# WU-CVGL/SIU3R

Measured on AMD Instinct MI355X. Metric: image-pairs/sec @2x512^2 (SIU3R network forward incl. panoptic post-process), higher is better.
Workload: dtype bf16x3 (fp32 activations, bf16 MFMA with hi/lo operand split; meets the 1e-3 parity bar)

## Files before the change

### siu3r_amd/csrc/gemm.hip

```cpp
#include <stdlib.h>

#include "common.h"
#include "gemm_epilogue.h"

int siu3r_gemm_dma_launch(const siu3r_gemm_params& p, int ni, void* stream);
int siu3r_gemm_dma_x3_launch(const siu3r_gemm_params& p, void* stream);
int siu3r_gemm_dma_mode(const siu3r_gemm_params& p);
int siu3r_gemm_dma_x3_mode(const siu3r_gemm_params& p);
int siu3r_gemm_pp_mode(const siu3r_gemm_params& p);
void siu3r_gemm_pp_name(const siu3r_gemm_params& p, int cfg, char* buf, int n);
int siu3r_gemm_pp_launch(const siu3r_gemm_params& p, int cfg, void* stream);
int siu3r_gemm_skinny_launch(const siu3r_gemm_params& p, void* stream);
bool siu3r_gemm_pp_folds_skinny(const siu3r_gemm_params& p);
bool siu3r_gemm_pp_a_x3_ok(const siu3r_gemm_params& p);
bool siu3r_gemm_pp_c_x3_ok(const siu3r_gemm_params& p, int cfg);
static const bool g_disable_dma = getenv("SIU3R_GEMM_NO_DMA") != nullptr;
static const int g_narrow_max = getenv("SIU3R_GEMM_NARROW_MAX") ? atoi(getenv("SIU3R_GEMM_NARROW_MAX")) : 0x7fffffff;

namespace {

constexpr int BM = 128, BK = 64;
constexpr int A_TILE_BYTES = BM * BK * 2;

__device__ __forceinline__ int lds_off(int row, int chunk) {
  return row * 128 + ((chunk ^ ((row >> 1) & 7)) << 4);
}

template <int A_F32, int SPLIT, int NI>
struct Regs {
  float4 ra0[A_F32 ? 4 : 1], ra1[A_F32 ? 4 : 1];
  uint4 rab[A_F32 ? 1 : 4];
  uint4 rwh[2 * NI], rwl[SPLIT ? 2 * NI : 1];
};

template <int A_F32, int SPLIT, int NI, bool LNF = false>
__global__ __launch_bounds__(256) void gemm_kernel(const siu3r_gemm_params p) {
  constexpr int BN = 64 * NI;
  constexpr int B_TILE_BYTES = BN * BK * 2;
  constexpr int PLANES = SPLIT ? 2 : 1;
  constexpr int STAGE_BYTES = PLANES * (A_TILE_BYTES + B_TILE_BYTES);
  constexpr int WROWS = 2 * NI;
  constexpr int SMEM_BYTES = 2 * STAGE_BYTES > siu3r_epi::staging_bytes<NI>() ? 2 * STAGE_BYTES : siu3r_epi::staging_bytes<NI>();
  __shared__ __attribute__((aligned(16))) unsigned char smem[SMEM_BYTES];

  const int t = threadIdx.x;
  const int lane = t & 63, wave = t >> 6;
// ... 236 lines not shown
  if (p.splitk <= 1 || NI != 1) p.splitk = 0;
  if (!p.w_lo && p.a_dtype == SIU3R_BF16 && p.a_mode != 2 && !g_disable_dma) {
    const int rc = siu3r_gemm_dma_launch(p, NI, s);
    if (rc <= 0) return rc;
  }
  if (p.w_x3 && NI == 1 && !g_disable_dma) {
    const int rc = siu3r_gemm_dma_x3_launch(p, s);
    if (rc <= 0) return rc;
  }
  p.splitk = 0;
  if (p.ln_stats) {
    if (p.w_lo) hipLaunchKernelGGL((gemm_kernel<1, 1, NI, true>), grid, block, 0, s, p);
    else if (p.a_dtype == SIU3R_F32) hipLaunchKernelGGL((gemm_kernel<1, 0, NI, true>), grid, block, 0, s, p);
    else hipLaunchKernelGGL((gemm_kernel<0, 0, NI, true>), grid, block, 0, s, p);
  } else if (p.w_lo) {
    hipLaunchKernelGGL((gemm_kernel<1, 1, NI>), grid, block, 0, s, p);
  } else if (p.a_dtype == SIU3R_F32) {
    hipLaunchKernelGGL((gemm_kernel<1, 0, NI>), grid, block, 0, s, p);
  } else {
    hipLaunchKernelGGL((gemm_kernel<0, 0, NI>), grid, block, 0, s, p);
  }
  SIU3R_LAUNCH_CHECK("siu3r_gemm");
  return 0;
}

}


static int g_tile_default = getenv("SIU3R_GEMM_PP") ? atoi(getenv("SIU3R_GEMM_PP")) : 0;
static int g_no_skinny = getenv("SIU3R_GEMM_NO_SKINNY") ? 1 : 0;
static int g_no_splitk = getenv("SIU3R_NO_SPLITK") ? atoi(getenv("SIU3R_NO_SPLITK")) : 0;
static int g_no_tuned = getenv("SIU3R_GEMM_NO_TUNED") ? 1 : 0;
static int g_force_skinny = getenv("SIU3R_GEMM_FORCE_SKINNY") ? 1 : 0;
static float g_bf16_pp_hurdle = getenv("SIU3R_GEMM_BF16_PP_HURDLE") ? (float)atof(getenv("SIU3R_GEMM_BF16_PP_HURDLE")) : 1.3f;
extern "C" int siu3r_gemm_tune(int key, int value) {
  if (key == 0) g_tile_default = value;
  else if (key == 1) g_no_skinny = value;
  else if (key == 2) g_no_splitk = value;
  else if (key == 3) g_no_tuned = value;
  else if (key == 4) g_force_skinny = value;
  else return 1;
  return 0;
}

#include "gemm_tuned.h"

namespace {
const siu3r_tuned_entry* tuned_entry(const siu3r_gemm_params& p, bool x3) {
  const int Z = p.batch > 0 ? p.batch : 1, ln = p.ln_stats ? 1 : 0;
  for (const siu3r_tuned_entry* e = kTuned; e->m; ++e)
    if (e->m == p.m && e->n == p.n && e->k == p.k && e->batch == Z && e->a_mode == p.a_mode && e->out_mode == p.out_mode && e->kh == p.kh &&
        e->stride == p.stride && e->x3 == (x3 ? 1 : 0) && e->ln == ln)
      return e;
  return nullptr;
}

struct Cand { int cfg, bm, bn, slots; float t0_x3, t_step_x3, t0_bf, t_step_bf; };
const Cand kCands[] = {{SIU3R_TILE_PP_256x256, 256, 256, 256, 16.3f, 1.18f, 12.1f, 0.80f},
                       {SIU3R_TILE_PP_256x128, 256, 128, 256, 11.7f, 0.65f, 8.5f, 0.47f},
                       {SIU3R_TILE_PP_128x128, 128, 128, 256, 7.8f, 0.40f, 6.5f, 0.30f},
                       {SIU3R_TILE_128x64, 128, 64, 512, 6.2f, 0.46f, 6.8f, 0.31f}};

void plan(const siu3r_gemm_params& p, siu3r_gemm_plan_t& pl) {
  memset(&pl, 0, sizeof(pl));
  const bool x3 = p.w_x3 != nullptr && p.a_dtype == SIU3R_F32;
  const int pp_mode = (g_disable_dma || p.a_mode == 2) ? -1 : siu3r_gemm_pp_mode(p);
  const int dma_mode = g_disable_dma ? -1 : (x3 ? siu3r_gemm_dma_x3_mode(p) : siu3r_gemm_dma_mode(p));
  int force = p.tile_cfg ? p.tile_cfg : g_tile_default;
  const bool may_split = !g_no_splitk && p.splitk != 1 && p.sk_ws && p.sk_cnt;
  int want_s = p.splitk;
  if (force == 0 && !g_no_tuned) {
    if (const siu3r_tuned_entry* e = tuned_entry(p, x3)) {
      force = e->tile_cfg;
      if (e->splitk > 0 && p.splitk == 0) want_s = (e->splitk > 1 && !may_split) ? 1 : e->splitk;
    }
  }
  const int64_t Z = p.batch > 0 ? p.batch : 1;
  const int ksteps = p.kpad / (x3 ? 16 : 32);
  float best_t = 0.f;
  int best = -1, best_s = 1, best_skinny = 0;
  for (int ci = 0; ci < 4; ++ci) {
    const Cand& c = kCands[ci];
    const bool is_pp = c.cfg > 0;
    if (is_pp && pp_mode < 0) continue;
    if (force != 0 && force != c.cfg && !(force > 0 && !is_pp && pp_mode < 0)) continue;
    const int rem = p.m % c.bm;
    const bool skinny_ok = is_pp && !g_no_skinny && p.a_mode == 0 && rem != 0 && rem <= 32 && p.n >= 64;
    for (int sk = (skinny_ok && g_force_skinny) ? 1 : 0; sk <= (skinny_ok ? 1 : 0); ++sk) {
      const int skinny = sk ? rem : 0;
      const int mrows = p.m - skinny;
      const int64_t tiles = (int64_t)((mrows + c.bm - 1) / c.bm) * ((p.n + c.bn - 1) / c.bn) * Z;
      const bool can_split = may_split && (is_pp || (dma_mode >= 0 && c.bn == 64));
      const bool fixed_s = want_s >= 1 && (want_s == 1 || can_split);
      const int smax = fixed_s ? want_s : (can_split ? 8 : 1);
      for (int S = (fixed_s ? want_s : 1); S <= smax; S *= 2) {
        if (S > 1) {
          if (ksteps / S < (is_pp ? 8 : 16) && !fixed_s) break;
          if (tiles * S * c.bm * c.bn > p.sk_ws_floats || tiles > p.sk_cnt_n) break;
          if (tiles >= 2 * c.slots && !fixed_s) break;
        }
        const int64_t wgs = tiles * S;
        const int64_t rounds = (wgs + c.slots - 1) / c.slots;
        float t = rounds * ((x3 ? c.t0_x3 : c.t0_bf) + (float)((ksteps + S - 1) / S) * (x3 ? c.t_step_x3 : c.t_step_bf));
        if (mrows == 0) t = 0.f;
        if (skinny && mrows > 0 && p.kpad <= 2048 && !getenv("SIU3R_GEMM_NO_FOLD")) t += 1.0f + (x3 ? 5.0f : 3.0f) * (float)p.kpad / 1024.f;
        else if (skinny) t += (skinny <= 4 && p.kpad >= 2048 && p.kpad <= 4096) ? 5.0f + (x3 ? 5.0f : 3.0f) * (float)p.kpad / 1024.f : 3.5f + (x3 ? 9.3f : 5.0f) * (float)p.kpad / 1024.f;
        if (S > 1) t += 2.5f + (float)(2.0 * S * tiles * c.bm * c.bn * 4.0 / 5.0e6);
        if (!x3 && is_pp && force == 0) t *= g_bf16_pp_hurdle;
        if (best < 0 || t < best_t) {
          best = ci;
          best_t = t;
          best_s = S;
          best_skinny = skinny;
        }
      }
    }
  }
  if (best < 0) best = 3;
  const Cand& c = kCands[best];
  pl.tile_cfg = c.cfg;
  pl.bm = c.bm;
  pl.bn = c.bn;
  pl.splitk = best_s;
  pl.skinny_rows = best_skinny;
  if (c.cfg < 0) {
    const int64_t tiles128 = (int64_t)((p.m + BM - 1) / BM) * ((p.n + 127) / 128) * Z;
    const bool narrow = (p.n <= 64) || (tiles128 < g_narrow_max && p.n > 64) || p.w_x3 != nullptr;
    pl.bn = narrow ? 64 : 128;
    if (!narrow || dma_mode < 0) pl.splitk = 1;
  }
  if (pl.splitk > 1) {
    const int64_t tiles = (int64_t)((p.m - pl.skinny_rows + pl.bm - 1) / pl.bm) * ((p.n + pl.bn - 1) / pl.bn) * Z;
    pl.ws_floats = tiles * pl.splitk * pl.bm * pl.bn;
    pl.counters = (int32_t)tiles;
  }
  auto tf = [](bool b) { return b ? "true" : "false"; };
  if (c.cfg > 0) {
    siu3r_gemm_pp_name(p, c.cfg, pl.kernel, sizeof(pl.kernel));
// ... 42 lines not shown
  SIU3R_CHECK(p.tile_cfg >= -1 && p.tile_cfg <= 3, "siu3r_gemm: bad tile_cfg %d", p.tile_cfg);
  if (p.bmod > 0) SIU3R_CHECK(p.batch > 0 && p.batch % p.bmod == 0, "siu3r_gemm: batch %d is not a multiple of bmod %d", p.batch, p.bmod);
  return 0;
}

extern "C" int siu3r_gemm_plan(const siu3r_gemm_params* pp, siu3r_gemm_plan_t* out) {
  SIU3R_CHECK(pp && out, "siu3r_gemm_plan: null argument");
  if (int rc = validate_gemm(*pp)) return rc;
  plan(*pp, *out);
  out->a_x3_ok = out->tile_cfg > 0 && siu3r_gemm_pp_a_x3_ok(*pp);
  out->c_x3_ok = out->tile_cfg > 0 && siu3r_gemm_pp_c_x3_ok(*pp, out->tile_cfg);
  return 0;
}

extern "C" int siu3r_gemm(const siu3r_gemm_params* pp, void* stream) {
  const siu3r_gemm_params& p = *pp;
  if (int rc = validate_gemm(p)) return rc;
  siu3r_gemm_plan_t pl;
  plan(p, pl);
  hipStream_t s = (hipStream_t)stream;
  SIU3R_CHECK(!p.a_x3 || (pl.tile_cfg > 0 && siu3r_gemm_pp_a_x3_ok(p)), "siu3r_gemm: a_x3 (pre-split A planes) needs a ping-pong plan, bf16x3 weights, dense A, "
              "k == kpad and lda / batch strides %% 32 == 0 (this block runs %s): query siu3r_gemm_plan_t.a_x3_ok first", pl.kernel);
  SIU3R_CHECK(!p.c_x3 || (pl.tile_cfg > 0 && siu3r_gemm_pp_c_x3_ok(p, pl.tile_cfg)), "siu3r_gemm: c_x3 (output planes) needs a ping-pong plan and the plain fp32 "
              "row-major output form with n %% 64 == 0, ldc / batch strides %% 32 == 0 (this block runs %s): query siu3r_gemm_plan_t.c_x3_ok first", pl.kernel);
  SIU3R_CHECK(p.c || p.c_x3, "siu3r_gemm: null output");
  siu3r_gemm_params q = p;
  q.splitk = pl.splitk;
  if (pl.splitk > 1) SIU3R_CHECK(p.sk_ws && p.sk_cnt && p.sk_ws_floats >= pl.ws_floats && p.sk_cnt_n >= pl.counters,
                                 "siu3r_gemm: split-K workspace too small (%ld floats / %d counters needed)", (long)pl.ws_floats, pl.counters);
  SIU3R_CHECK(!(p.splitk > 1 && pl.splitk != p.splitk), "siu3r_gemm: splitk=%d was requested but %s cannot split K for this problem (it would run %d slice(s)); "
              "request 0 / 1 or another tile_cfg", p.splitk, pl.kernel, pl.splitk);
  if (pl.tile_cfg > 0) {
    q.m_main = pl.skinny_rows > 0 ? p.m - pl.skinny_rows : 0;
    if (!(pl.skinny_rows > 0 && q.m_main == 0)) {
      const int rc = siu3r_gemm_pp_launch(q, pl.tile_cfg, stream);
      if (rc) return rc;
    }
    if (pl.skinny_rows > 0 && !(q.m_main > 0 && siu3r_gemm_pp_folds_skinny(q))) {
      q.splitk = 0;
      return siu3r_gemm_skinny_launch(q, stream);
    }
    return 0;
  }
  return pl.bn == 64 ? launch<1>(q, s) : launch<2>(q, s);
}
```

### siu3r_amd/csrc/gemm_pp.hip

```cpp
#include "gemm_pp_kernel.h"

namespace siu3r_gemm_pp {
template <bool X3, bool LNF>
__global__ __launch_bounds__(512, 2) void gemm_skinny_kernel(const siu3r_gemm_params p) {
#if __HIP_DEVICE_COMPILE__
  __shared__ __attribute__((aligned(16))) unsigned char smem[SKINNY_SMEM_BYTES];
  skinny_rows_body<X3, LNF>(p, smem, blockIdx.x, blockIdx.z);
#endif
}

constexpr int GV_ROWS = 4, GV_KMAX = 4096;
template <bool X3, bool LNF>
__global__ __launch_bounds__(512) void gemm_skinny_gemv_kernel(const siu3r_gemm_params p) {
#if __HIP_DEVICE_COMPILE__
  constexpr int ESZ = X3 ? 4 : 2;
  __shared__ __attribute__((aligned(16))) float s_a[GV_ROWS * GV_KMAX];
  __shared__ __attribute__((aligned(16))) float s_res[GV_ROWS][64];
  __shared__ __attribute__((aligned(16))) unsigned char s_stage[siu3r_epi_pp::WAVE_STAGE_BYTES];
  const int t = threadIdx.x, lane = t & 63;
  const int wave = __builtin_amdgcn_readfirstlane(t >> 6);
  const int M = p.m, N = p.n, K = p.k, kpad = p.kpad;
  const int row0 = p.m_main, R = M - row0, col0 = blockIdx.x * 64, z = blockIdx.z;
  const siu3r_zoff zof = siu3r_batch_offsets(p, z);
  const unsigned char* Ab = (const unsigned char*)p.a + zof.a * ESZ;
// ... 132 lines not shown
  return p.relu_in ? -1 : 2;
}

void siu3r_gemm_pp_name(const siu3r_gemm_params& p, int cfg, char* buf, int n) {
  const bool x3 = p.w_x3 != nullptr && p.a_dtype == SIU3R_F32;
  const int mode = siu3r_gemm_pp_mode(p);
  snprintf(buf, n, "siu3r_gemm_pp::gemm_pp_kernel<%s, %d, %d, %d, %s, %s%s>", x3 ? "true" : "false", cfg == 3 ? 1 : 2, cfg == 1 ? 4 : 2, mode,
           (mode == 1 && p.relu_in) ? "true" : "false", (mode == 0 && p.ln_stats) ? "true" : "false", (x3 && mode <= 1 && p.a_x3) ? ", true" : "");
}

bool siu3r_gemm_pp_a_x3_ok(const siu3r_gemm_params& p) {
  const bool x3 = p.w_x3 != nullptr && p.a_dtype == SIU3R_F32;
  if (!x3 || ((uintptr_t)p.a % 16) != 0 || p.sa % 32 != 0 || p.sa_i % 32 != 0) return false;
  const int mode = siu3r_gemm_pp_mode(p);
  if (mode == 0) return p.k == p.kpad && p.lda % 32 == 0;
  return mode == 1 && p.cin % 32 == 0 && !p.relu_in;
}
bool siu3r_gemm_pp_c_x3_ok(const siu3r_gemm_params& p, int cfg) {
  if (siu3r_epi_pp::g_force_general || siu3r_gemm_pp_mode(p) < 0) return false;
  const int MI_ = cfg == 3 ? 1 : 2;
  const int64_t res_b = p.r_dtype == SIU3R_F32 ? 4 : 2;
  const bool res_ok = !p.residual || (p.r_dtype == SIU3R_F32 && (p.ldr * res_b) % 16 == 0 && ((uintptr_t)p.residual % 16) == 0 && (p.sr * res_b) % 16 == 0 &&
                                       (p.sr_i * res_b) % 16 == 0 && (int64_t)(32 * MI_) * p.ldr < (1 << 28));
  const bool up_ok = !p.up_src || (p.up_dtype == SIU3R_F32 && ((uintptr_t)p.up_src % 16) == 0 && (int64_t)p.m * p.n < (1 << 29));
  return p.out_mode == 0 && up_ok && !p.c_aux && p.c_dtype == SIU3R_F32 && p.n % 64 == 0 && (int64_t)(32 * MI_) * p.ldc < (1 << 28) && res_ok &&
         p.ldc % 32 == 0 && p.sc % 32 == 0 && p.sc_i % 32 == 0 && ((uintptr_t)p.c % 16) == 0 && ((uintptr_t)p.c_x3 % 16) == 0 &&
         p.c_x3_col0 >= 0 && p.c_x3_col0 % 64 == 0;
}

static const bool g_no_fold = getenv("SIU3R_GEMM_NO_FOLD") != nullptr;
bool siu3r_gemm_pp_folds_skinny(const siu3r_gemm_params& p) {
  return !g_no_fold && p.m_main > 0 && p.m_main < p.m && p.a_mode == 0 && p.kpad <= 2048 && siu3r_gemm_pp_mode(p) == 0;
}

int siu3r_gemm_pp_launch(const siu3r_gemm_params& pin, int cfg, void* stream) {
  using namespace siu3r_gemm_pp;
  siu3r_gemm_params p = pin;
  const bool x3 = p.w_x3 != nullptr && p.a_dtype == SIU3R_F32;
  const int mode = siu3r_gemm_pp_mode(p);
  if (mode < 0) return 1;
  const int MI_ = cfg == 3 ? 1 : 2, NJ_ = cfg == 1 ? 4 : 2;
  const int bm = 128 * MI_, bn = 64 * NJ_;
  const int mrows = p.m_main > 0 ? p.m_main : p.m;
  const int tm = (mrows + bm - 1) / bm, tn = (p.n + bn - 1) / bn;
  int best = -1;
  long best_cost = 0;
  for (int gx = 1; gx <= 8; gx *= 2) {
    const int gy = 8 / gx;
    const int rm = (tm + gy - 1) / gy, rn = (tn + gx - 1) / gx;
    const long cost = (long)rm * rn * 1000000 + (long)rm * bm + (long)rn * bn;
    if (best < 0 || cost < best_cost) {
      best = gx;
      best_cost = cost;
    }
  }
  p.map_gx = best;
  p.map_rm = (tm + (8 / best) - 1) / (8 / best);
  p.map_rn = (tn + best - 1) / best;
  dim3 grid(8 * p.map_rm * p.map_rn, p.splitk > 1 ? p.splitk : 1, p.batch > 0 ? p.batch : 1), block(512);
  p.sk_gx = 0;
  if (siu3r_gemm_pp_folds_skinny(p)) {
    p.sk_gx = (int)grid.x;
    grid.x += (unsigned)((p.n + 63) / 64);
  }
  hipStream_t s = (hipStream_t)stream;
  const bool lnf = p.ln_stats != nullptr;
#ifdef SIU3R_PP_MINI
  hipLaunchKernelGGL((gemm_pp_kernel<SIU3R_PP_MINI, false, false>), grid, block, 0, s, p);
#else
  if (cfg == 1) (x3 ? siu3r_gemm_pp_go_t1x : siu3r_gemm_pp_go_t1b)(p, mode, lnf, grid, s);
  else if (cfg == 2) (x3 ? siu3r_gemm_pp_go_t2x : siu3r_gemm_pp_go_t2b)(p, mode, lnf, grid, s);
  else (x3 ? siu3r_gemm_pp_go_t3x : siu3r_gemm_pp_go_t3b)(p, mode, lnf, grid, s);
#endif
  SIU3R_LAUNCH_CHECK("siu3r_gemm(pp)");
  return 0;
}

int siu3r_gemm_skinny_launch(const siu3r_gemm_params& p, void* stream) {
  using namespace siu3r_gemm_pp;
  const bool x3 = p.w_x3 != nullptr && p.a_dtype == SIU3R_F32;
  dim3 grid((p.n + 63) / 64, 1, p.batch > 0 ? p.batch : 1), block(512);
  hipStream_t s = (hipStream_t)stream;
  const bool lnf = p.ln_stats != nullptr;
#ifndef SIU3R_PP_MINI
  const int rows = p.m - p.m_main, esz = x3 ? 4 : 2;
  static const bool no_gemv = getenv("SIU3R_GEMM_NO_GEMV") != nullptr;
  if (!no_gemv && rows >= 1 && rows <= GV_ROWS && p.kpad >= 2048 && p.kpad <= GV_KMAX && p.k % 4 == 0 && ((int64_t)p.lda * esz) % 16 == 0 &&
      ((uintptr_t)p.a % 16) == 0 && (p.sa * esz) % 16 == 0 && (p.sa_i * esz) % 16 == 0) {
    if (x3 && lnf) hipLaunchKernelGGL((gemm_skinny_gemv_kernel<true, true>), grid, block, 0, s, p);
    else if (x3) hipLaunchKernelGGL((gemm_skinny_gemv_kernel<true, false>), grid, block, 0, s, p);
    else if (lnf) hipLaunchKernelGGL((gemm_skinny_gemv_kernel<false, true>), grid, block, 0, s, p);
    else hipLaunchKernelGGL((gemm_skinny_gemv_kernel<false, false>), grid, block, 0, s, p);
    SIU3R_LAUNCH_CHECK("siu3r_gemm(skinny gemv)");
    return 0;
// ... 10 lines not shown
```

### siu3r_amd/csrc/gemm_pp_kernel.h

```cpp
#pragma once
#include <stdlib.h>

#include "common.h"
#include "gemm_epilogue_pp.h"

#ifndef SIU3R_PP_SCHED
#define SIU3R_PP_SCHED 0
#endif

namespace siu3r_gemm_pp {

constexpr unsigned OOB = 0xffffff00u;
constexpr int RSRC_FLAGS = 0x00020000;
constexpr int nstage(int MI, int NJ) { return (MI == 2 && NJ == 4) ? 4 : (MI == 2 ? 6 : 8); }
constexpr int spp(int MI, int NJ) { return (MI == 2 && NJ == 4) ? 1 : 2; }

typedef __attribute__((address_space(3))) void* lds_ptr;
typedef __attribute__((ext_vector_type(4))) unsigned int u32x4;
typedef __attribute__((ext_vector_type(2))) short i16x2;

template <int MI, int NJ>
constexpr int smem_bytes() {
  constexpr int ring = nstage(MI, NJ) * (128 * MI + 64 * NJ) * 64, st = siu3r_epi_pp::staging_bytes();
  return ring > st ? ring : st;
}

#define SIU3R_DS_READ(dst, addr, OFF) asm volatile("ds_read_b128 %0, %1 offset:%2" : "=v"(dst) : "v"(addr), "i"(OFF) : "memory")

constexpr int SKINNY_SMEM_BYTES = 8 * 8192 + siu3r_epi_pp::WAVE_STAGE_BYTES;
template <bool X3, bool LNF>
__device__ __forceinline__ void skinny_rows_body(const siu3r_gemm_params& p, unsigned char* smem, int colgroup, int z) {
#if __HIP_DEVICE_COMPILE__
  constexpr int ESZ = X3 ? 4 : 2;
  const int t = threadIdx.x, lane = t & 63;
  const int wave = __builtin_amdgcn_readfirstlane(t >> 6);
  const int l31 = lane & 31, lh = lane >> 5;
  const int M = p.m, N = p.n, K = p.k, kpad = p.kpad;
  const int row0 = p.m_main, col0 = colgroup * 64;
  const siu3r_zoff zof = siu3r_batch_offsets(p, z);
  const unsigned char* Ab = (const unsigned char*)p.a + zof.a * ESZ;
  const unsigned char* Wb = X3 ? (const unsigned char*)p.w_x3 + zof.w * 4 : (const unsigned char*)p.w_hi + zof.w * 2;
  const int WROW = X3 ? kpad * 4 : kpad * 2;
  __amdgpu_buffer_rsrc_t rA = __builtin_amdgcn_make_buffer_rsrc((void*)Ab, (short)0, (int)(((int64_t)(M - 1) * p.lda + K) * ESZ), RSRC_FLAGS);
  __amdgpu_buffer_rsrc_t rW = __builtin_amdgcn_make_buffer_rsrc((void*)Wb, (short)0, (int)((int64_t)N * WROW), RSRC_FLAGS);
  int m = row0 + l31;
  if (m > M - 1) m = M - 1;
  const unsigned a_voff = (unsigned)((int64_t)m * p.lda * ESZ + lh * (8 * ESZ));
  const bool aps = X3 && p.a_x3 != 0;
  const unsigned a_voff_ps = (unsigned)((int64_t)m * p.lda * ESZ + lh * 16);
  unsigned w_voff[2];
#pragma unroll
  for (int j = 0; j < 2; ++j) {
    int n = col0 + j * 32 + l31;
    if (n > N - 1) n = N - 1;
    w_voff[j] = (unsigned)((int64_t)n * WROW + lh * 16);
  }
// ... 79 lines not shown
  }
  __syncthreads();
  if (wave != 0) return;
#pragma unroll 1
  for (int w = 1; w < 8; ++w) {
#pragma unroll
    for (int j = 0; j < 2; ++j)
#pragma unroll
      for (int qv = 0; qv < 4; ++qv) {
        const float4 v = *(const float4*)(part + ((w * 8 + j * 4 + qv) * 64 + lane) * 4);
        acc[0][j][4 * qv] += v.x;
        acc[0][j][4 * qv + 1] += v.y;
        acc[0][j][4 * qv + 2] += v.z;
        acc[0][j][4 * qv + 3] += v.w;
      }
  }
  siu3r_epi_pp::wave_rows<1, 2, LNF>(p, acc, (float*)(smem + 8 * 8192), row0, col0, M, z, lane);
#endif
}

template <bool X3, int MI, int NJ, int MODE, bool RELU, bool LNF, bool APS = false>
__global__ __launch_bounds__(512, 2) void gemm_pp_kernel(const siu3r_gemm_params p) {
#if __HIP_DEVICE_COMPILE__
  constexpr int BM = 128 * MI, BN = 64 * NJ;
  constexpr int NSTAGE = nstage(MI, NJ), SPP = spp(MI, NJ), PD = NSTAGE - SPP;
  static_assert(NSTAGE % SPP == 0, "a phase uses whole stages");
  constexpr int STAGE_BYTES = (BM + BN) * 64;
  constexpr int A_PCS = MI, W_PCS = NJ / 2, PPW = A_PCS + W_PCS;
  constexpr int ESZ = X3 ? 4 : 2;
  constexpr int KSTEP = X3 ? 16 : 32;
  constexpr int CK = 16 / ESZ;
  static_assert(NJ % 2 == 0, "W pieces are dealt to whole waves");
  static_assert(!APS || (X3 && MODE <= 1 && !RELU), "pre-split A: bf16x3, dense rows or the tap-cursor gather (cin % 32 == 0)");
  __shared__ __attribute__((aligned(1024))) unsigned char smem[smem_bytes<MI, NJ>()];
  static_assert(smem_bytes<MI, NJ>() >= SKINNY_SMEM_BYTES, "the folded remainder-row workgroups use the ring's LDS");

  if constexpr (MODE == 0) {
    if (p.sk_gx > 0 && (int)blockIdx.x >= p.sk_gx) {
      const int cg = (int)blockIdx.x - p.sk_gx;
      if (blockIdx.y == 0 && cg * 64 < p.n) skinny_rows_body<X3, LNF>(p, smem, cg, blockIdx.z);
      return;
    }
  }

  const int t = threadIdx.x;
  const int lane = t & 63;
  const int wave = __builtin_amdgcn_readfirstlane(t >> 6);
  const int grp = wave >> 2;
  const int wm = wave & 3, wn = grp;
  const int l31 = lane & 31, lh = lane >> 5;

  const int M = p.m_main > 0 ? p.m_main : p.m;
  const int N = p.n, K = p.k, kpad = p.kpad;
  const int tiles_m = (M + BM - 1) / BM, tiles_n = (N + BN - 1) / BN;
  const int xcd = (blockIdx.x + blockIdx.z) & 7, li = blockIdx.x >> 3;
  const int map_gx = p.map_gx;
  const int ry = xcd / map_gx, rx = xcd - ry * map_gx;
  const int lm = li / p.map_rn, ln = li - lm * p.map_rn;
  const int tile_m = ry * p.map_rm + lm, tile_n = rx * p.map_rn + ln;
  if (lm >= p.map_rm || tile_m >= tiles_m || tile_n >= tiles_n) return;
  const int z = blockIdx.z;
  const int np_all = kpad / (KSTEP * SPP);
  const int pbase = p.splitk > 1 ? (int)((int64_t)blockIdx.y * np_all / p.splitk) : 0;
  const int np = p.splitk > 1 ? (int)((int64_t)(blockIdx.y + 1) * np_all / p.splitk) - pbase : np_all;
  const int sbase = pbase * SPP, ns = np * SPP;

  const siu3r_zoff zof = siu3r_batch_offsets(p, z);
  const unsigned char* Ab = (const unsigned char*)p.a + zof.a * ESZ;
  const unsigned char* Wb = X3 ? (const unsigned char*)p.w_x3 + zof.w * 4 : (const unsigned char*)p.w_hi + zof.w * 2;
  const int WROW = X3 ? kpad * 4 : kpad * 2;

  const int prow = lane >> 2;
  const int q = (lane & 3) ^ ((lane >> 4) & 3);
  const int cin = p.cin, iw = p.iw, ih = p.ih, kw = p.kw, kh = p.kh;
  const int pad_bias = (MODE != 0) ? (p.pad * iw + p.pad) * cin * ESZ : 0;
  __amdgpu_buffer_rsrc_t rA, rW;
  if (MODE == 0)
    rA = __builtin_amdgcn_make_buffer_rsrc((void*)Ab, (short)0, (int)(((int64_t)(p.m - 1) * p.lda + K) * ESZ), RSRC_FLAGS);
  else
    rA = __builtin_amdgcn_make_buffer_rsrc((void*)(Ab - pad_bias), (short)0, (int)OOB, RSRC_FLAGS);
  rW = __builtin_amdgcn_make_buffer_rsrc((void*)Wb, (short)0, (int)((int64_t)N * WROW), RSRC_FLAGS);

  unsigned a_voff[A_PCS], a_mask[A_PCS];
  int a_iy0[A_PCS], a_ix0[A_PCS];
#pragma unroll
  for (int i = 0; i < A_PCS; ++i) {
    const int r = (wave * A_PCS + i) * 16 + prow;
    int m = tile_m * BM + r;
    const bool row_ok = m < M;
    if (!row_ok) m = M - 1;
    a_voff[i] = a_mask[i] = 0;
    a_iy0[i] = a_ix0[i] = 0;
    if (MODE == 0) {
      a_voff[i] = (unsigned)((int64_t)m * p.lda * ESZ + q * 16 + ((APS && q >= 2) ? 32 : 0));
    } else {
      const int ohw = p.oh * p.ow;
      const int b = m / ohw, rr = m - b * ohw;
      const int oy = rr / p.ow, ox = rr - oy * p.ow;
      const int iy0 = oy * p.stride - p.pad, ix0 = ox * p.stride - p.pad;
      if (MODE == 1) {
        a_voff[i] = (unsigned)((((b * ih + iy0) * iw + ix0) * cin) * ESZ + q * 16 + ((APS && q >= 2) ? 32 : 0) + pad_bias);
        unsigned mk = 0;
        for (int ky = 0; ky < kh; ++ky)
          for (int kx = 0; kx < kw; ++kx)
            if (iy0 + ky >= 0 && iy0 + ky < ih && ix0 + kx >= 0 && ix0 + kx < iw) mk |= 1u << (ky * kw + kx);
        a_mask[i] = row_ok ? mk : 0u;
      } else {
        a_voff[i] = (unsigned)((((b * ih + iy0) * iw + ix0) * cin) * ESZ + pad_bias);
        a_iy0[i] = row_ok ? iy0 : -(1 << 20);
        a_ix0[i] = ix0;
      }
    }
  }
  unsigned w_voff[W_PCS];
#pragma unroll
  for (int i = 0; i < W_PCS; ++i) {
    const int r = (wave * W_PCS + i) * 16 + prow;
    int n = tile_n * BN + r;
    if (n > N - 1) n = N - 1;
    w_voff[i] = (unsigned)((int64_t)n * WROW + q * 16 + ((X3 && q >= 2) ? 32 : 0));
  }
  const bool ktail = kpad > K;
  const int ks_tail0 = K / KSTEP;

  int cur_c0 = 0, cur_kx = 0, cur_toff = 0, cur_row = 0;
  unsigned cur_bit = 1u;
  auto cursor_advance = [&]() {
    cur_c0 += KSTEP;
    cur_toff += APS ? ((cur_c0 & 16) ? 32 : 96) : KSTEP * ESZ;
    if (cur_c0 == cin) {
      cur_c0 = 0;
      cur_bit <<= 1;
      if (++cur_kx == kw) {
        cur_kx = 0;
        cur_row += iw * cin * ESZ;
      }
      cur_toff = cur_row + cur_kx * cin * ESZ;
    }
  };
  int s_c0 = 0, s_kx = 0, s_ky = 0;
  int qs_r = 0, qs_qx = 0, qs_qy = 0;
  if (MODE == 2) {
    const int qq = KSTEP / cin;
    qs_r = KSTEP - qq * cin;
    qs_qy = qq / kw;
    qs_qx = qq - qs_qy * kw;
    const int k0 = q * CK;
    const int tap = k0 / cin;
    s_c0 = k0 - tap * cin;
    s_ky = tap / kw;
    s_kx = tap - s_ky * kw;
  }
  auto state_advance = [&]() {
    s_c0 += qs_r;
    const int carry = s_c0 >= cin ? 1 : 0;
    s_c0 -= carry * cin;
// ... 4 lines not shown
  };

  auto issue_piece = [&](int s, int stage, int k) {
    const int sg = sbase + (s < ns ? s : ns - 1);
    unsigned char* dstA = smem + stage * STAGE_BYTES + wave * (A_PCS * 1024);
    unsigned char* dstW = smem + stage * STAGE_BYTES + BM * 64 + wave * (W_PCS * 1024);
    if (k < A_PCS) {
      const int i = k;
      if (MODE == 0 && APS) {
        __builtin_amdgcn_raw_ptr_buffer_load_lds(rA, (lds_ptr)(dstA + i * 1024), 16, a_voff[i], (sg >> 1) * 128 + (sg & 1) * 32, 0, 0);
      } else if (MODE == 0) {
        unsigned voff = a_voff[i];
        if (ktail && sg >= ks_tail0) voff = (sg * KSTEP + q * CK < K) ? voff : OOB;
        __builtin_amdgcn_raw_ptr_buffer_load_lds(rA, (lds_ptr)(dstA + i * 1024), 16, voff, sg * 64, 0, 0);
      } else if (MODE == 1) {
        const unsigned voff = (a_mask[i] & cur_bit) ? a_voff[i] : OOB;
        __builtin_amdgcn_raw_ptr_buffer_load_lds(rA, (lds_ptr)(dstA + i * 1024), 16, voff, cur_toff, 0, 0);
      } else {
        const int iy = a_iy0[i] + s_ky, ix = a_ix0[i] + s_kx;
        const bool ok = s_ky < kh && (unsigned)iy < (unsigned)ih && (unsigned)ix < (unsigned)iw;
        const unsigned voff = ok ? a_voff[i] + (unsigned)(((s_ky * iw + s_kx) * cin + s_c0) * ESZ) : OOB;
        __builtin_amdgcn_raw_ptr_buffer_load_lds(rA, (lds_ptr)(dstA + i * 1024), 16, voff, 0, 0, 0);
      }
    } else {
      const int i = k - A_PCS;
      const int soffW = X3 ? (sg >> 1) * 128 + (sg & 1) * 32 : sg * 64;
      __builtin_amdgcn_raw_ptr_buffer_load_lds(rW, (lds_ptr)(dstW + i * 1024), 16, w_voff[i], soffW, 0, 0);
    }
    if (k == PPW - 1) {
      if (MODE == 1 && s + 1 < ns) cursor_advance();
      if (MODE == 2 && s + 1 < ns) state_advance();
    }
  };
  auto issue = [&](int s, int stage) {
#pragma unroll
    for (int k = 0; k < PPW; ++k) issue_piece(s, stage, k);
  };

  f32x16 acc[MI][NJ];
#pragma unroll
  for (int i = 0; i < MI; ++i)
#pragma unroll
    for (int j = 0; j < NJ; ++j)
#pragma unroll
      for (int r = 0; r < 16; ++r) acc[i][j][r] = 0.f;

  const unsigned int lds_base = (unsigned int)(size_t)(__attribute__((address_space(3))) unsigned char*)smem;
  const int fsw = (l31 >> 2) & 3;
  const unsigned int rowA = (wm * (32 * MI) + l31) * 64, rowB = BM * 64 + (wn * (32 * NJ) + l31) * 64;
  const unsigned int offA0 = rowA + ((((X3 && !APS) ? 2 * lh : lh) ^ fsw) << 4), offA1 = rowA + ((((X3 && !APS) ? 2 * lh + 1 : 2 + lh) ^ fsw) << 4);
  const unsigned int offB0 = rowB + ((lh ^ fsw) << 4), offB1 = rowB + (((2 + lh) ^ fsw) << 4);

  u32x4 fa[SPP][MI][2], fb[SPP][NJ][2];
  auto read_frags = [&](int u, int stage) {
    const unsigned int sb = lds_base + stage * STAGE_BYTES;
    const unsigned int a0 = sb + offA0, a1 = sb + offA1, b0 = sb + offB0, b1 = sb + offB1;
#define SIU3R_RD_A(I) if constexpr (I < MI) { SIU3R_DS_READ(fa[u][I][0], a0, I * 2048); SIU3R_DS_READ(fa[u][I][1], a1, I * 2048); }
#define SIU3R_RD_B(J) if constexpr (J < NJ) { SIU3R_DS_READ(fb[u][J][0], b0, J * 2048); SIU3R_DS_READ(fb[u][J][1], b1, J * 2048); }
    SIU3R_RD_A(0) SIU3R_RD_A(1)
    SIU3R_RD_B(0) SIU3R_RD_B(1) SIU3R_RD_B(2) SIU3R_RD_B(3)
#undef SIU3R_RD_A
#undef SIU3R_RD_B
  };
  auto wait_frags = [&]() {
    asm volatile("s_waitcnt lgkmcnt(0)" ::: "memory");
#pragma unroll
    for (int u = 0; u < SPP; ++u) {
#pragma unroll
      for (int i = 0; i < MI; ++i) asm volatile("" : "+v"(fa[u][i][0]), "+v"(fa[u][i][1]));
#pragma unroll
      for (int j = 0; j < NJ; ++j) asm volatile("" : "+v"(fb[u][j][0]), "+v"(fb[u][j][1]));
    }
  };
  auto as_frag = [&](u32x4 v) {
    if (!X3 && RELU) {
#pragma unroll
      for (int e = 0; e < 4; ++e) {
        union { unsigned int u; i16x2 h; } x;
        x.u = v[e];
        x.h = __builtin_elementwise_max(x.h, (i16x2){0, 0});
        v[e] = x.u;
      }
    }
    union { u32x4 u; bf16x8 h; } cv;
    cv.u = v;
    return cv.h;
  };

#ifndef SIU3R_PP_DBG
#define SIU3R_PP_DBG 0
#endif
  constexpr int dbg = SIU3R_PP_DBG;
  constexpr bool dma = !(dbg & 1);
  unsigned tsum[8] = {0, 0, 0, 0, 0, 0, 0, 0}, tlast = 0;
  auto tick = [&](int seg) {
    if constexpr ((dbg & 64) != 0) {
      const unsigned now = (unsigned)__builtin_readcyclecounter();
      tsum[seg] += now - tlast;
      tlast = now;
    }
  };

  for (int s_ = 0; s_ < sbase; ++s_) {
    if (MODE == 1) cursor_advance();
    if (MODE == 2) state_advance();
  }
  constexpr int YOUNG = (PD - SPP) * PPW;
  auto wait_young = [&]() {
    static_assert(YOUNG == 8 || YOUNG == 6, "vmcnt immediate");
    if constexpr (YOUNG == 8) asm volatile("s_waitcnt vmcnt(8)" ::: "memory");
    else asm volatile("s_waitcnt vmcnt(6)" ::: "memory");
  };
  constexpr bool IMF = SIU3R_PP_SCHED == 1;
  const int pd_grp = (IMF && grp == 1) ? PD + SPP : PD;
#pragma unroll
  for (int s_ = 0; s_ < PD; ++s_) issue(s_, s_);
  if (IMF && grp == 1) {
#pragma unroll
    for (int s_ = PD; s_ < PD + SPP; ++s_) issue(s_, s_);
    static_assert(PD * PPW == 12, "vmcnt immediate");
    asm volatile("s_waitcnt vmcnt(12)" ::: "memory");
  } else {
    wait_young();
  }
  __builtin_amdgcn_s_barrier();
  asm volatile("" ::: "memory");
  if (grp == 1) __builtin_amdgcn_s_barrier();
  if constexpr ((dbg & 64) != 0) tlast = (unsigned)__builtin_readcyclecounter();

  int st_rd = 0, st_is = pd_grp % NSTAGE;
  auto mf_hook = [&](int s, int u, int c) {
    if constexpr (IMF) {
      constexpr int TOT = (X3 ? 3 : 2) * MI * NJ;
#pragma unroll
      for (int k = 0; k < PPW; ++k)
        if (dma && c == ((2 * k + 1) * TOT) / (2 * PPW) + 1) {
          issue_piece(s + pd_grp + u, st_is + u, k);
          __builtin_amdgcn_sched_barrier(0);
        }
    }
  };
  for (int s = 0; s < ns; s += SPP) {
    tick(7);
#pragma unroll
    for (int u = 0; u < SPP; ++u)
      if (!(dbg & 4)) read_frags(u, st_rd + u);
    if (dma && !IMF) {
#pragma unroll
      for (int u = 0; u < SPP; ++u) issue(s + PD + u, st_is + u);
    }
    __builtin_amdgcn_sched_barrier(0);
    tick(1);
    wait_frags();
    tick(2);
    if (grp == 1 && dma) wait_young();
    __builtin_amdgcn_sched_barrier(0);
    if (!(dbg & 16)) __builtin_amdgcn_s_barrier();
    __builtin_amdgcn_sched_barrier(0);
    tick(4);
    __builtin_amdgcn_s_setprio(1);
#pragma unroll
    for (int u = 0; u < SPP; ++u) {
      bf16x8 bh[NJ][2];
#pragma unroll
      for (int j = 0; j < NJ; ++j) {
        union { u32x4 u; bf16x8 h; } c0, c1;
        c0.u = fb[u][j][0];
        c1.u = fb[u][j][1];
        bh[j][0] = c0.h;
        bh[j][1] = c1.h;
      }
      if constexpr ((dbg & 2) != 0) {
#pragma unroll
        for (int i = 0; i < MI; ++i) asm volatile("" :: "v"(fa[u][i][0]), "v"(fa[u][i][1]));
#pragma unroll
        for (int j = 0; j < NJ; ++j) asm volatile("" :: "v"(bh[j][0]), "v"(bh[j][1]));
      } else if constexpr (X3) {
        union U8 { u32x4 u; bf16x8 h; };
        U8 ah[MI], al[MI];
        auto raw = [&](int i, int e) { return e < 4 ? fa[u][i][0][e] : fa[u][i][1][e - 4]; };
        auto relu = [&](unsigned int x) { return (RELU && (x & 0x80000000u)) ? 0u : x; };
        auto hi_pair = [&](int i, int e) { ah[i].u[e] = __builtin_amdgcn_perm(relu(raw(i, 2 * e + 1)), relu(raw(i, 2 * e)), 0x07060302u); };
// ... 18 lines not shown
        constexpr int NM = MI * NJ;
        constexpr int NP = 4 * MI;
#pragma unroll
        for (int g = 0; g < 2 * NM; ++g) {
          const int r = g / NM, ij = g % NM, i = ij / NJ, j = ij % NJ;
          acc[i][j] = __builtin_amdgcn_mfma_f32_32x32x16_bf16(ah[i].h, bh[j][r], acc[i][j], 0, 0, 0);
          mf_hook(s, u, g + 1);
          if constexpr (!nosplit) {
            const int p0 = g * NP / (2 * NM), p1 = (g + 1) * NP / (2 * NM);
#pragma unroll
            for (int pp = p0; pp < p1; ++pp) lo_pair(pp / 4, pp % 4);
          }
          if ((g & 1) == 1) __builtin_amdgcn_sched_barrier(0);
        }
#pragma unroll
        for (int i = 0; i < MI; ++i)
#pragma unroll
          for (int j = 0; j < NJ; ++j) {
            acc[i][j] = __builtin_amdgcn_mfma_f32_32x32x16_bf16(al[i].h, bh[j][0], acc[i][j], 0, 0, 0);
            mf_hook(s, u, 2 * NM + i * NJ + j + 1);
          }
      } else {
#pragma unroll
        for (int ks = 0; ks < 2; ++ks)
#pragma unroll
          for (int i = 0; i < MI; ++i)
#pragma unroll
            for (int j = 0; j < NJ; ++j) {
              acc[i][j] = __builtin_amdgcn_mfma_f32_32x32x16_bf16(as_frag(fa[u][i][ks]), bh[j][ks], acc[i][j], 0, 0, 0);
              mf_hook(s, u, (ks * MI + i) * NJ + j + 1);
            }
      }
    }
    __builtin_amdgcn_s_setprio(0);
    __builtin_amdgcn_sched_barrier(0);
    tick(5);
    if (grp == 0 && dma) wait_young();
    __builtin_amdgcn_sched_barrier(0);
    if (!(dbg & 16)) __builtin_amdgcn_s_barrier();
    __builtin_amdgcn_sched_barrier(0);
    tick(6);
    st_rd = (st_rd + SPP == NSTAGE) ? 0 : st_rd + SPP;
    st_is = (st_is + SPP == NSTAGE) ? 0 : st_is + SPP;
  }
  if (grp == 0) __builtin_amdgcn_s_barrier();
  asm volatile("s_waitcnt vmcnt(0)" ::: "memory");
  __builtin_amdgcn_s_barrier();
  asm volatile("" ::: "memory");
  if constexpr ((dbg & 64) != 0) {
    if (p.trace && (t & 255) == 0) {
      uint64_t* tr = p.trace + ((size_t)blockIdx.x * 2 + grp) * 8;
#pragma unroll
      for (int e = 0; e < 8; ++e) tr[e] = tsum[e];
    }
  }
  if (dbg & 32) {
    float keep = 0.f;
#pragma unroll
    for (int i = 0; i < MI; ++i)
#pragma unroll
      for (int j = 0; j < NJ; ++j)
#pragma unroll
        for (int r = 0; r < 16; ++r) keep += acc[i][j][r];
    if (keep == 123.456f) ((float*)p.c)[0] = 1.f;
    return;
  }
  if (p.splitk > 1) {
    const int64_t tile_id = ((int64_t)z * tiles_m + tile_m) * tiles_n + tile_n;
    if (!siu3r_epi_pp::splitk_reduce<MI, NJ>(p, acc, smem, tile_id, t)) return;
  }
  siu3r_epi_pp::wave_rows<MI, NJ, LNF>(p, acc, (float*)(smem + wave * siu3r_epi_pp::WAVE_STAGE_BYTES), tile_m * BM + wm * (32 * MI),
                                       tile_n * BN + wn * (32 * NJ), M, z, lane);
#endif
}


}
```

Measured before the change: 54.04.

## Carry skinny remainder rows inside last ping-pong GEMM tile via extra MFMA

When M leaves at most 16 remainder rows, the workgroups on the last M-tile now also stream the final 16 A rows into a small extra LDS ring. They accumulate those rows with 16x16 MFMAs alongside the main tile and write them out in an extra epilogue. This replaces the separate skinny kernel launch or the folded extra workgroups. The grid mapping also gains an optional tail layout that maps the partial last tile row separately, and the planner's cost model is updated for the carry path. The trade-off is more LDS, extra vmcnt bookkeeping and extra work on the tail workgroups.

```diff
diff --git a/siu3r_amd/csrc/gemm.hip b/siu3r_amd/csrc/gemm.hip
--- a/siu3r_amd/csrc/gemm.hip
+++ b/siu3r_amd/csrc/gemm.hip
@@ -12,6 +12,7 @@
 int siu3r_gemm_pp_launch(const siu3r_gemm_params& p, int cfg, void* stream);
 int siu3r_gemm_skinny_launch(const siu3r_gemm_params& p, void* stream);
 bool siu3r_gemm_pp_folds_skinny(const siu3r_gemm_params& p);
+bool siu3r_gemm_pp_carries(const siu3r_gemm_params& p, int cfg, int rem, int splitk);
 bool siu3r_gemm_pp_a_x3_ok(const siu3r_gemm_params& p);
 bool siu3r_gemm_pp_c_x3_ok(const siu3r_gemm_params& p, int cfg);
 static const bool g_disable_dma = getenv("SIU3R_GEMM_NO_DMA") != nullptr;
@@ -314,6 +315,7 @@
 static int g_no_splitk = getenv("SIU3R_NO_SPLITK") ? atoi(getenv("SIU3R_NO_SPLITK")) : 0;
 static int g_no_tuned = getenv("SIU3R_GEMM_NO_TUNED") ? 1 : 0;
 static int g_force_skinny = getenv("SIU3R_GEMM_FORCE_SKINNY") ? 1 : 0;
+extern int g_gemm_no_carry;
 static float g_bf16_pp_hurdle = getenv("SIU3R_GEMM_BF16_PP_HURDLE") ? (float)atof(getenv("SIU3R_GEMM_BF16_PP_HURDLE")) : 1.3f;
 extern "C" int siu3r_gemm_tune(int key, int value) {
   if (key == 0) g_tile_default = value;
@@ -321,6 +323,7 @@
   else if (key == 2) g_no_splitk = value;
   else if (key == 3) g_no_tuned = value;
   else if (key == 4) g_force_skinny = value;
+  else if (key == 5) g_gemm_no_carry = value;
   else return 1;
   return 0;
 }
@@ -385,7 +388,8 @@
         const int64_t rounds = (wgs + c.slots - 1) / c.slots;
         float t = rounds * ((x3 ? c.t0_x3 : c.t0_bf) + (float)((ksteps + S - 1) / S) * (x3 ? c.t_step_x3 : c.t_step_bf));
         if (mrows == 0) t = 0.f;
-        if (skinny && mrows > 0 && p.kpad <= 2048 && !getenv("SIU3R_GEMM_NO_FOLD")) t += 1.0f + (x3 ? 5.0f : 3.0f) * (float)p.kpad / 1024.f;
+        if (skinny && mrows > 0 && !g_force_skinny && siu3r_gemm_pp_carries(p, c.cfg, skinny, S)) t += 1.0f + 0.0625f * (float)ksteps * (x3 ? c.t_step_x3 : c.t_step_bf);
+        else if (skinny && mrows > 0 && p.kpad <= 2048 && !getenv("SIU3R_GEMM_NO_FOLD")) t +=1.0f + (x3 ? 5.0f : 3.0f) * (float)p.kpad / 1024.f;
         else if (skinny) t += (skinny <= 4 && p.kpad >= 2048 && p.kpad <= 4096) ? 5.0f + (x3 ? 5.0f : 3.0f) * (float)p.kpad / 1024.f : 3.5f + (x3 ? 9.3f : 5.0f) * (float)p.kpad / 1024.f;
         if (S > 1) t += 2.5f + (float)(2.0 * S * tiles * c.bm * c.bn * 4.0 / 5.0e6);
         if (!x3 && is_pp && force == 0) t *= g_bf16_pp_hurdle;
@@ -494,11 +498,13 @@
               "request 0 / 1 or another tile_cfg", p.splitk, pl.kernel, pl.splitk);
   if (pl.tile_cfg > 0) {
     q.m_main = pl.skinny_rows > 0 ? p.m - pl.skinny_rows : 0;
+    const bool carry = q.m_main > 0 && !g_force_skinny && siu3r_gemm_pp_carries(q, pl.tile_cfg, pl.skinny_rows, pl.splitk);
+    q.sk_gx = carry ? -1 : 0;
     if (!(pl.skinny_rows > 0 && q.m_main == 0)) {
       const int rc = siu3r_gemm_pp_launch(q, pl.tile_cfg, stream);
       if (rc) return rc;
     }
-    if (pl.skinny_rows > 0 && !(q.m_main > 0 && siu3r_gemm_pp_folds_skinny(q))) {
+    if (pl.skinny_rows > 0 && !carry && !(q.m_main > 0 && siu3r_gemm_pp_folds_skinny(q))) {
       q.splitk = 0;
       return siu3r_gemm_skinny_launch(q, stream);
     }
diff --git a/siu3r_amd/csrc/gemm_pp.hip b/siu3r_amd/csrc/gemm_pp.hip
--- a/siu3r_amd/csrc/gemm_pp.hip
+++ b/siu3r_amd/csrc/gemm_pp.hip
@@ -188,6 +188,11 @@
 bool siu3r_gemm_pp_folds_skinny(const siu3r_gemm_params& p) {
   return !g_no_fold && p.m_main > 0 && p.m_main < p.m && p.a_mode == 0 && p.kpad <= 2048 && siu3r_gemm_pp_mode(p) == 0;
 }
+int g_gemm_no_carry = getenv("SIU3R_GEMM_NO_CARRY") ? 1 : 0;
+bool siu3r_gemm_pp_carries(const siu3r_gemm_params& p, int cfg, int rem, int splitk) {
+  return !g_gemm_no_carry && (cfg == 2 || cfg == 3) && rem > 0 && rem <= 16 && splitk <= 1 && p.a_mode == 0 && p.m - rem >= 128 &&
+         siu3r_gemm_pp_mode(p) == 0;
+}
 
 int siu3r_gemm_pp_launch(const siu3r_gemm_params& pin, int cfg, void* stream) {
   using namespace siu3r_gemm_pp;
@@ -199,23 +204,31 @@
   const int bm = 128 * MI_, bn = 64 * NJ_;
   const int mrows = p.m_main > 0 ? p.m_main : p.m;
   const int tm = (mrows + bm - 1) / bm, tn = (p.n + bn - 1) / bn;
-  int best = -1;
+  const bool carry = p.sk_gx < 0;
+  const int tm_full = mrows / bm;
+  const bool tail_ok = !g_gemm_no_carry && tm_full >= 1 && tm > tm_full && mrows - tm_full * bm <= 32;
+  int best = -1, best_tail = 0;
   long best_cost = 0;
-  for (int gx = 1; gx <= 8; gx *= 2) {
-    const int gy = 8 / gx;
-    const int rm = (tm + gy - 1) / gy, rn = (tn + gx - 1) / gx;
-    const long cost = (long)rm * rn * 1000000 + (long)rm * bm + (long)rn * bn;
-    if (best < 0 || cost < best_cost) {
-      best = gx;
-      best_cost = cost;
-    }
-  }
+  for (int tail = 0; tail <= (tail_ok ? 1 : 0); ++tail)
+    for (int gx = 1; gx <= 8; gx *= 2) {
+      const int gy = 8 / gx, rows = tail ? tm_full : tm;
+      if (tail && rows % gy != 0) continue;
+      const int rm = (rows + gy - 1) / gy, rn = (tn + gx - 1) / gx, extra = tail ? (rn + gy - 1) / gy : 0;
+      const long cost = (long)(rm * rn + extra) * 1000000 + (long)rm * bm + (long)rn * bn;
+      if (best < 0 || cost < best_cost) {
+        best = gx;
+        best_tail = tail;
+        best_cost = cost;
+      }
+    }
+  const int gy = 8 / best, map_rows = best_tail ? tm_full : tm;
   p.map_gx = best;
-  p.map_rm = (tm + (8 / best) - 1) / (8 / best);
+  p.map_rm = (map_rows + gy - 1) / gy;
   p.map_rn = (tn + best - 1) / best;
-  dim3 grid(8 * p.map_rm * p.map_rn, p.splitk > 1 ? p.splitk : 1, p.batch > 0 ? p.batch : 1), block(512);
-  p.sk_gx = 0;
-  if (siu3r_gemm_pp_folds_skinny(p)) {
+  const int per_region = p.map_rm * p.map_rn + (best_tail ? (p.map_rn + gy - 1) / gy : 0);
+  dim3 grid(8 * per_region, p.splitk > 1 ? p.splitk : 1, p.batch > 0 ? p.batch : 1), block(512);
+  p.sk_gx = carry ? -1 : 0;
+  if (!carry && siu3r_gemm_pp_folds_skinny(p)) {
     p.sk_gx = (int)grid.x;
     grid.x += (unsigned)((p.n + 63) / 64);
   }
diff --git a/siu3r_amd/csrc/gemm_pp_kernel.h b/siu3r_amd/csrc/gemm_pp_kernel.h
--- a/siu3r_amd/csrc/gemm_pp_kernel.h
+++ b/siu3r_amd/csrc/gemm_pp_kernel.h
@@ -19,9 +19,11 @@
 typedef __attribute__((ext_vector_type(4))) unsigned int u32x4;
 typedef __attribute__((ext_vector_type(2))) short i16x2;
 
-template <int MI, int NJ>
+constexpr bool carry_tile(int MI, int NJ) { return spp(MI, NJ) == 2 && NJ == 2; }
+template <int MI, int NJ, int MODE = 1>
 constexpr int smem_bytes() {
-  constexpr int ring = nstage(MI, NJ) * (128 * MI + 64 * NJ) * 64, st = siu3r_epi_pp::staging_bytes();
+  constexpr int ring = nstage(MI, NJ) * (128 * MI + 64 * NJ) * 64 + ((MODE == 0 && carry_tile(MI, NJ)) ? nstage(MI, NJ) * 1024 : 0);
+  constexpr int st = siu3r_epi_pp::staging_bytes();
   return ring > st ? ring : st;
 }
 
@@ -167,8 +169,10 @@
   constexpr int CK = 16 / ESZ;
   static_assert(NJ % 2 == 0, "W pieces are dealt to whole waves");
   static_assert(!APS || (X3 && MODE <= 1 && !RELU), "pre-split A: bf16x3, dense rows or the tap-cursor gather (cin % 32 == 0)");
-  __shared__ __attribute__((aligned(1024))) unsigned char smem[smem_bytes<MI, NJ>()];
-  static_assert(smem_bytes<MI, NJ>() >= SKINNY_SMEM_BYTES, "the folded remainder-row workgroups use the ring's LDS");
+  __shared__ __attribute__((aligned(1024))) unsigned char smem[smem_bytes<MI, NJ, MODE>()];
+  static_assert(smem_bytes<MI, NJ, MODE>() >= SKINNY_SMEM_BYTES, "the folded remainder-row workgroups use the ring's LDS");
+  constexpr bool CARRY_T = MODE == 0 && carry_tile(MI, NJ) && SIU3R_PP_SCHED == 0;
+  constexpr int RING_BYTES = NSTAGE * STAGE_BYTES;
 
   if constexpr (MODE == 0) {
     if (p.sk_gx > 0 && (int)blockIdx.x >= p.sk_gx) {
@@ -191,9 +195,10 @@
   const int xcd = (blockIdx.x + blockIdx.z) & 7, li = blockIdx.x >> 3;
   const int map_gx = p.map_gx;
   const int ry = xcd / map_gx, rx = xcd - ry * map_gx;
-  const int lm = li / p.map_rn, ln = li - lm * p.map_rn;
-  const int tile_m = ry * p.map_rm + lm, tile_n = rx * p.map_rn + ln;
-  if (lm >= p.map_rm || tile_m >= tiles_m || tile_n >= tiles_n) return;
+  const int in_reg = p.map_rm * p.map_rn, gy = 8 / map_gx;
+  const int lm = li < in_reg ? li / p.map_rn : p.map_rm, ln = li < in_reg ? li - lm * p.map_rn : (li - in_reg) * gy + ry;
+  const int tile_m = li < in_reg ? ry * p.map_rm + lm : tiles_m - 1, tile_n = rx * p.map_rn + ln;
+  if ((li < in_reg && lm >= p.map_rm) || ln >= p.map_rn || tile_m >= tiles_m || tile_n >= tiles_n) return;
   const int z = blockIdx.z;
   const int np_all = kpad / (KSTEP * SPP);
   const int pbase = p.splitk > 1 ? (int)((int64_t)blockIdx.y * np_all / p.splitk) : 0;
@@ -257,6 +262,9 @@
   }
   const bool ktail = kpad > K;
   const int ks_tail0 = K / KSTEP;
+  const bool carry = CARRY_T && p.sk_gx < 0 && tile_m == tiles_m - 1;
+  const bool carry_dma = carry && wave == 0;
+  const unsigned c_voff = (unsigned)((int64_t)(p.m - 16 + prow) * p.lda * ESZ + q * 16 + ((APS && q >= 2) ? 32 : 0));
 
   int cur_c0 = 0, cur_kx = 0, cur_toff = 0, cur_row = 0;
   unsigned cur_bit = 1u;
@@ -327,9 +335,25 @@
       if (MODE == 2 && s + 1 < ns) state_advance();
     }
   };
-  auto issue = [&](int s, int stage) {
+  auto issue_carry = [&](int s, int stage) {
+    if constexpr (CARRY_T) {
+      if (carry_dma) {
+        const int sg = sbase + (s < ns ? s : ns - 1);
+        lds_ptr dst = (lds_ptr)(smem + RING_BYTES + stage * 1024);
+        if (APS) {
+          __builtin_amdgcn_raw_ptr_buffer_load_lds(rA, dst, 16, c_voff, (sg >> 1) * 128 + (sg & 1) * 32, 0, 0);
+        } else {
+          unsigned voff = c_voff;
+          if (ktail && sg >= ks_tail0) voff = (sg * KSTEP + q * CK < K) ? voff : OOB;
+          __builtin_amdgcn_raw_ptr_buffer_load_lds(rA, dst, 16, voff, sg * 64, 0, 0);
+        }
+      }
+    }
+  };
+  auto issue = [&](int s, int stage, bool with_carry) {
 #pragma unroll
     for (int k = 0; k < PPW; ++k) issue_piece(s, stage, k);
+    if (with_carry) issue_carry(s, stage);
   };
 
   f32x16 acc[MI][NJ];
@@ -347,6 +371,29 @@
   const unsigned int offB0 = rowB + ((lh ^ fsw) << 4), offB1 = rowB + (((2 + lh) ^ fsw) << 4);
 
   u32x4 fa[SPP][MI][2], fb[SPP][NJ][2];
+  u32x4 fc[2], fd[2];
+  f32x4 acc_c = {0.f, 0.f, 0.f, 0.f};
+  const int cg = lane >> 4, cr = lane & 15, csw = (cr >> 2) & 3;
+  const unsigned int offC = (unsigned)RING_BYTES + cr * 64, offD = BM * 64 + (wave * 16 + cr) * 64;
+  auto read_carry = [&](int stage) {
+    if constexpr (CARRY_T) {
+      if constexpr (X3) {
+        const int st = stage + (cg >> 1), h = cg & 1;
+        const unsigned int c0 = lds_base + st * 1024 + offC, d0 = lds_base + st * STAGE_BYTES + offD;
+        const unsigned int ca = c0 + ((((APS ? h : 2 * h)) ^ csw) << 4), cb = c0 + ((((APS ? 2 + h : 2 * h + 1)) ^ csw) << 4);
+        SIU3R_DS_READ(fc[0], ca, 0);
+        SIU3R_DS_READ(fc[1], cb, 0);
+        SIU3R_DS_READ(fd[0], d0 + ((h ^ csw) << 4), 0);
+        SIU3R_DS_READ(fd[1], d0 + (((2 + h) ^ csw) << 4), 0);
+      } else {
+#pragma unroll
+        for (int u = 0; u < 2; ++u) {
+          SIU3R_DS_READ(fc[u], lds_base + (stage + u) * 1024 + offC + ((cg ^ csw) << 4), 0);
+          SIU3R_DS_READ(fd[u], lds_base + (stage + u) * STAGE_BYTES + offD + ((cg ^ csw) << 4), 0);
+        }
+      }
+    }
+  };
   auto read_frags = [&](int u, int stage) {
     const unsigned int sb = lds_base + stage * STAGE_BYTES;
     const unsigned int a0 = sb + offA0, a1 = sb + offA1, b0 = sb + offB0, b1 = sb + offB1;
@@ -366,6 +413,7 @@
 #pragma unroll
       for (int j = 0; j < NJ; ++j) asm volatile("" : "+v"(fb[u][j][0]), "+v"(fb[u][j][1]));
     }
+    if (CARRY_T && carry) asm volatile("" : "+v"(fc[0]), "+v"(fc[1]), "+v"(fd[0]), "+v"(fd[1]));
   };
   auto as_frag = [&](u32x4 v) {
     if (!X3 && RELU) {
@@ -401,18 +449,26 @@
     if (MODE == 2) state_advance();
   }
   constexpr int YOUNG = (PD - SPP) * PPW;
+  constexpr int YOUNG_C = (PD - SPP) * (PPW + 1);
   auto wait_young = [&]() {
     static_assert(YOUNG == 8 || YOUNG == 6, "vmcnt immediate");
-    if constexpr (YOUNG == 8) asm volatile("s_waitcnt vmcnt(8)" ::: "memory");
-    else asm volatile("s_waitcnt vmcnt(6)" ::: "memory");
+    static_assert(!CARRY_T || YOUNG_C == 8 || YOUNG_C == 12, "vmcnt immediate");
+    if (CARRY_T && carry_dma) {
+      if constexpr (YOUNG_C == 12) asm volatile("s_waitcnt vmcnt(12)" ::: "memory");
+      else asm volatile("s_waitcnt vmcnt(8)" ::: "memory");
+    } else if constexpr (YOUNG == 8) {
+      asm volatile("s_waitcnt vmcnt(8)" ::: "memory");
+    } else {
+      asm volatile("s_waitcnt vmcnt(6)" ::: "memory");
+    }
   };
   constexpr bool IMF = SIU3R_PP_SCHED == 1;
   const int pd_grp = (IMF && grp == 1) ? PD + SPP : PD;
 #pragma unroll
-  for (int s_ = 0; s_ < PD; ++s_) issue(s_, s_);
+  for (int s_ = 0; s_ < PD; ++s_) issue(s_, s_, true);
   if (IMF && grp == 1) {
 #pragma unroll
-    for (int s_ = PD; s_ < PD + SPP; ++s_) issue(s_, s_);
+    for (int s_ = PD; s_ < PD + SPP; ++s_) issue(s_, s_, true);
     static_assert(PD * PPW == 12, "vmcnt immediate");
     asm volatile("s_waitcnt vmcnt(12)" ::: "memory");
   } else {
@@ -434,15 +490,22 @@
           __builtin_amdgcn_sched_barrier(0);
         }
     }
+    if constexpr (CARRY_T && !IMF) {
+      if (dma && c == 2) {
+        issue_carry(s + PD + u, st_is + u);
+        __builtin_amdgcn_sched_barrier(0);
+      }
+    }
   };
   for (int s = 0; s < ns; s += SPP) {
     tick(7);
 #pragma unroll
     for (int u = 0; u < SPP; ++u)
       if (!(dbg & 4)) read_frags(u, st_rd + u);
+    if (CARRY_T && carry) read_carry(st_rd);
     if (dma && !IMF) {
 #pragma unroll
-      for (int u = 0; u < SPP; ++u) issue(s + PD + u, st_is + u);
+      for (int u = 0; u < SPP; ++u) issue(s + PD + u, st_is + u, false);
     }
     __builtin_amdgcn_sched_barrier(0);
     tick(1);
@@ -527,6 +590,33 @@
             }
       }
     }
+    if constexpr (CARRY_T) {
+      if (carry) {
+        union U8 { u32x4 u; bf16x8 h; };
+        U8 a0, a1, b0, b1;
+        b0.u = fd[0];
+        b1.u = fd[1];
+        if constexpr (X3 && !APS) {
+#pragma unroll
+          for (int e = 0; e < 4; ++e) {
+            const unsigned int x0 = e < 2 ? fc[0][2 * e] : fc[1][2 * e - 4], x1 = e < 2 ? fc[0][2 * e + 1] : fc[1][2 * e - 3];
+            a0.u[e] = __builtin_amdgcn_perm(x1, x0, 0x07060302u);
+            a1.u[e] = pack_bf16x2(__uint_as_float(x0) - __uint_as_float(x0 & 0xffff0000u), __uint_as_float(x1) - __uint_as_float(x1 & 0xffff0000u));
+          }
+        } else {
+          a0.u = fc[0];
+          a1.u = fc[1];
+        }
+        if constexpr (X3) {
+          acc_c = __builtin_amdgcn_mfma_f32_16x16x32_bf16(a0.h, b0.h, acc_c, 0, 0, 0);
+          acc_c = __builtin_amdgcn_mfma_f32_16x16x32_bf16(a0.h, b1.h, acc_c, 0, 0, 0);
+          acc_c = __builtin_amdgcn_mfma_f32_16x16x32_bf16(a1.h, b0.h, acc_c, 0, 0, 0);
+        } else {
+          acc_c = __builtin_amdgcn_mfma_f32_16x16x32_bf16(a0.h, b0.h, acc_c, 0, 0, 0);
+          acc_c = __builtin_amdgcn_mfma_f32_16x16x32_bf16(a1.h, b1.h, acc_c, 0, 0, 0);
+        }
+      }
+    }
     __builtin_amdgcn_s_setprio(0);
     __builtin_amdgcn_sched_barrier(0);
     tick(5);
@@ -566,6 +656,28 @@
   }
   siu3r_epi_pp::wave_rows<MI, NJ, LNF>(p, acc, (float*)(smem + wave * siu3r_epi_pp::WAVE_STAGE_BYTES), tile_m * BM + wm * (32 * MI),
                                        tile_n * BN + wn * (32 * NJ), M, z, lane);
+  if constexpr (CARRY_T) {
+    if (carry) {
+      constexpr int LDB = BN + 4;
+      float* blk = (float*)smem;
+      __syncthreads();
+#pragma unroll
+      for (int i = 0; i < 4; ++i) blk[(4 * cg + i) * LDB + wave * 16 + cr] = acc_c[i];
+      __syncthreads();
+      const int R = p.m - M, col0 = tile_n * BN + wave * 64;
+      if (wave < BN / 64 && col0 < N) {
+        f32x16 out[1][2];
+#pragma unroll
+        for (int j = 0; j < 2; ++j)
+#pragma unroll
+          for (int i = 0; i < 16; ++i) {
+            const int r = 8 * (i >> 2) + 4 * lh + (i & 3);
+            out[0][j][i] = r < R ? blk[(r + 16 - R) * LDB + wave * 64 + j * 32 + l31] : 0.f;
+          }
+        siu3r_epi_pp::wave_rows<1, 2, LNF>(p, out, (float*)(smem + 16 * LDB * 4 + wave * siu3r_epi_pp::WAVE_STAGE_BYTES), M, col0, p.m, z, lane);
+      }
+    }
+  }
 #endif
 }
 
```

Result: no change. 54.23, median of 6 (+0.3%).
